# YifanXu74/MQ-Det

Measured on AMD Instinct MI355X. Metric: images/sec MQ-GLIP-T 800×1333 5-shot vision queries, 1/2/4/8 MI355X, higher is better.
Workload: dtype f16; 1 GPU; BASELINE.json configs[1]: MQ-GLIP-T (Swin-T + BERT-base + GCP + 6-layer VLDyHead), 5 vision queries x 40 classes, 141-token caption, LVIS-style post-processing; every step a full forward (feature / language caches OFF; only host-side tokenizer / query-selection results are memoised)); global_batch=8, batch_per_gpu=8, image=800x1333 -> 800x1344, parallelism=dp1, weights=seeded random init (no checkpoints offline), residual_streams=fp32

## Files before the change

### include/mqdet_hip.h

```cpp
#ifndef MQDET_HIP_H
#define MQDET_HIP_H
#ifdef __cplusplus
extern "C" {
#endif

int mq_abi_version(void);

long mq_attn_workspace_bytes(int B, int H, int Nq, int D, int nsplit);
int mq_attn_fwd(const void* q, const void* k, const void* vt, void* o, const float* key_bias, const int* kv_len,
                const unsigned char* qk_mask, long mask_bs, long mask_hs, long mask_rs, void* workspace,
                int B, int H, int Nq, int Nk, int D,
                long q_bs, long q_rs, long q_hs, long k_bs, long k_rs, long k_hs, long vt_bs, long vt_rs, long vt_hs,
                long o_bs, long o_rs, long bias_bs, long bias_hs, float scale, float clamp, int nsplit, void* stream);

int mq_attn_resident_fwd(const void* q, const void* k, const void* vt, void* o, const float* key_bias, const int* kv_len,
                         const unsigned char* qk_mask, long mask_bs, long mask_hs, long mask_rs, int B, int H, int Nq, int Nk, int D,
                         long q_bs, long q_rs, long q_hs, long k_bs, long k_rs, long k_hs, long vt_bs, long vt_rs, long vt_hs,
                         long o_bs, long o_rs, long bias_bs, long bias_hs, float scale, float clamp, void* stream);

int mq_attn_chunked_fwd(const void* q, const void* k, const void* vt, void* o, const float* key_bias, const int* kv_len,
                        void* workspace, int B, int H, int Nq, int Nk, int D,
                        long q_bs, long q_rs, long q_hs, long k_bs, long k_rs, long k_hs, long vt_bs, long vt_rs, long vt_hs,
                        long o_bs, long o_rs, long bias_bs, long bias_hs, float scale, float clamp, int nsplit, void* stream);

// ... 12 lines not shown
                      const void* out_bias, void* out, int B, int N, int T, int heads, int max_kv, float clamp, int variant,
                      void* stream);

long mq_vlfuse_t2i_workspace_bytes(int B, int T, int nsplit);
int mq_vlfuse_t2i_fwd(const void* kf, long kv_bs, long kv_hs, long kv_ts, const void* v_ln, const int* kv_len, const unsigned char* key_mask,
                      long key_mask_bs, void* workspace, void* out, int B, int N, int T, int heads, int nsplit, int max_kv, float clamp, int variant,
                      void* stream);

int mq_layernorm_fwd(const void* x, int x_f32, const void* res, int res_f32, const void* gamma, const void* beta, void* y,
                     float* y32, void* xsum, long rows, int C, float eps, void* stream);

int mq_layernorm2_fwd(const void* x, int x_f32, const void* res, int res_f32, const void* gamma, const void* beta, void* y,
                     float* y32, void* xsum, long rows, int C, float eps, void* stream);
int mq_layernorm_clamp_fwd(const void* x, int x_f32, const void* res, int res_f32, const void* gamma, const void* beta, void* y, float* y32,
                           void* xsum, long rows, int C, float eps, float clamp, void* stream);
int mq_clamp_gelu_clamp(const void* x, void* out, long n, float clamp, void* stream);

int mq_patch_merge_ln_fwd(const void* x, int x_f32, const void* gamma, const void* beta, void* y, int B, int H, int W, int C, float eps,
                          void* stream);

int mq_swin_mlp2_fwd(const float* x, const void* delta, const void* ln_g, const void* ln_b, float eps, const void* w1f,
                     const void* b1, const void* w2f, const void* b2, float* out, const void* next_g, const void* next_b,
                     float eps_next, void* y, long M, int C, int flags, void* stream);

int mq_conv3x3_fwd(const void* x, const void* w, const void* bias, void* out, int B, int H, int W, int C, long x_bs,
                   int N, int out_ld, int stride, void* stream);
int mq_conv3x3_nchw32_fwd(const void* x, const void* w, const void* bias, float* out, int B, int H, int W, int C, long x_bs,
                          int N, void* stream);

int mq_conv3x3_nchw32_v2_fwd(const void* x, const void* w, const void* bias, float* out, int B, int H, int W, int C, long x_bs,
                          int N, void* stream);
typedef struct mq_conv_level {
  const void* x; float* out; long x_bs; int H, W;
} mq_conv_level;
int mq_conv3x3_nchw32_group_fwd(const mq_conv_level* levels, int nl, const void* w, const void* bias, int B, int C, int N, void* stream);
int mq_pool2x2_tokens_fwd(const mq_conv_level* levels, int nl, void* out, int B, int C, void* stream);
int mq_dcnv2_stats_blocks(int H, int W, int stride);
typedef struct mq_dcn_branch {
  const void* x; const float* om; const void* w; const void* bias; void* out; float* stats; const float* wy; const float* wx;
  long x_bs;
  int B, H, W, C, oH, oW, N, out_ld, stride, flags;
} mq_dcn_branch;
int mq_dcnv2_group_fwd(const mq_dcn_branch* branches, int n, void* stream);
int mq_dcnv2_fwd(const void* x, const float* om, const void* w, const void* bias, void* out, float* stats, const float* wy,
                 const float* wx, int B, int H, int W, int C, long x_bs, int oH, int oW, int N, int out_ld, int stride,
                 int flags, void* stream);
// ... 102 lines not shown
#define MQ_BF16_TWIN(name) extern decltype(name) name##_bf16;
#else
#define MQ_BF16_TWIN(name) extern __typeof__(name) name##_bf16;
#endif
MQ_BF16_TWIN(mq_attn_fwd)
MQ_BF16_TWIN(mq_attn_resident_fwd)
MQ_BF16_TWIN(mq_attn_text_fwd)
MQ_BF16_TWIN(mq_bert_attn_qkv_fwd)
MQ_BF16_TWIN(mq_patch_embed_fwd)
MQ_BF16_TWIN(mq_attn_chunked_fwd)
MQ_BF16_TWIN(mq_window_attn_fwd)
MQ_BF16_TWIN(mq_window_attn_qkv_fwd)
MQ_BF16_TWIN(mq_gcp_sparse_attn_fwd)
MQ_BF16_TWIN(mq_gcp_gate_residual_fwd)
MQ_BF16_TWIN(mq_gcp_attn_fwd)
MQ_BF16_TWIN(mq_vlfuse_i2t_fwd)
MQ_BF16_TWIN(mq_vlfuse_t2i_fwd)
MQ_BF16_TWIN(mq_layernorm_fwd)
MQ_BF16_TWIN(mq_layernorm2_fwd)
MQ_BF16_TWIN(mq_layernorm_clamp_fwd)
MQ_BF16_TWIN(mq_clamp_gelu_clamp)
MQ_BF16_TWIN(mq_patch_merge_ln_fwd)
MQ_BF16_TWIN(mq_swin_mlp2_fwd)
MQ_BF16_TWIN(mq_conv3x3_fwd)
MQ_BF16_TWIN(mq_conv3x3_nchw32_fwd)
MQ_BF16_TWIN(mq_conv3x3_nchw32_v2_fwd)
MQ_BF16_TWIN(mq_conv3x3_nchw32_group_fwd)
MQ_BF16_TWIN(mq_dcnv2_fwd)
MQ_BF16_TWIN(mq_dcnv2_group_fwd)
MQ_BF16_TWIN(mq_dyconv_stats)
MQ_BF16_TWIN(mq_dyconv_coef)
MQ_BF16_TWIN(mq_dyconv_coef_group)
MQ_BF16_TWIN(mq_dyconv_fuse)
MQ_BF16_TWIN(mq_dyrelu_coef)
MQ_BF16_TWIN(mq_dyconv_epilogue_group)
MQ_BF16_TWIN(mq_dyrelu_apply)
MQ_BF16_TWIN(mq_add_upsample_nearest)
MQ_BF16_TWIN(mq_pool2x2_tokens_fwd)
MQ_BF16_TWIN(mq_dyrelu_ln_fwd)
MQ_BF16_TWIN(mq_align_scores_fwd)
MQ_BF16_TWIN(mq_align_fused_fwd)
MQ_BF16_TWIN(mq_box_decode)
MQ_BF16_TWIN(mq_roi_align_fwd)
MQ_BF16_TWIN(mq_msdeform_attn_fwd)
MQ_BF16_TWIN(mq_msdeform_attn_q_fwd)

// ... 51 lines not shown
```

### mq_det_amd/build.py

```python
import os
import subprocess
import sys

HERE = os.path.dirname(os.path.abspath(__file__))
CSRC = os.path.join(HERE, "csrc")
LIB_DIR = os.path.join(HERE, "lib")
LIB = os.path.join(LIB_DIR, "libmqdet_hip.so")
SOURCES = ["api.hip", "attn.hip", "attn_resident.hip", "attn_text.hip", "bert_attn.hip", "vlfuse_attn.hip", "window_attn.hip", "patch_embed.hip", "gcp.hip", "gcp_fused.hip", "conv_igemm.hip", "conv_small.hip", "conv_small2.hip", "conv_small3.hip", "dcn_fused.hip", "layernorm.hip", "layernorm2.hip", "dyconv.hip", "post.hip", "post2.hip", "align_fused.hip", "nms2.hip", "roi_align.hip", "swin_mlp2.hip", "msda.hip", "tta.hip", "lvis_eval.hip", "query_bank.hip"]
F32_SKIP = ("roi_align.hip", "nms2.hip", "post2.hip", "tta.hip", "lvis_eval.hip", "query_bank.hip")
FLAGS = ["--offload-arch=gfx950", "-O3", "-std=c++17", "-fPIC"]
EXTRA_FLAGS = {"dcn_fused.hip": ["-fno-slp-vectorize"],
               "swin_mlp2.hip": ["-fno-slp-vectorize"],
               "attn_resident.hip": ["-fno-slp-vectorize", "-mllvm", "-amdgpu-mfma-vgpr-form"],
               "attn_text.hip": ["-fno-slp-vectorize", "-mllvm", "-amdgpu-mfma-vgpr-form"],
               "bert_attn.hip": ["-fno-slp-vectorize", "-mllvm", "-amdgpu-mfma-vgpr-form"]}


STAMP = os.path.join(LIB_DIR, "libmqdet_hip.stamp")


def _digest():
    import hashlib
    h = hashlib.sha256()
    deps = sorted(os.path.join(CSRC, f) for f in os.listdir(CSRC)) + [os.path.join(HERE, "..", "include", "mqdet_hip.h"), os.path.abspath(__file__)]
    for d in deps:
        if os.path.isfile(d):
            with open(d, "rb") as f:
                h.update(os.path.basename(d).encode() + b"\0" + f.read())
    return h.hexdigest()


def _stale():
    if not os.path.exists(LIB) or not os.path.exists(STAMP):
        return True
    with open(STAMP) as f:
# ... 36 lines not shown
```

### mq_det_amd/modeling/pipeline.py

```python
import math
import os

import torch
import torch.nn.functional as F

from .. import ops

NEG = -1.0e30


def _pack_swin(P, sd, SW, p, device, dtype):
    def h(name):
        return sd[name].detach().to(device=device, dtype=dtype).contiguous()
    ws = SW.WINDOW_SIZE
    N = ws * ws
    for i, (depth, heads) in enumerate(zip(SW.DEPTHS, SW.NUM_HEADS)):
        for j in range(depth):
            b = f"{p}.layers.{i}.blocks.{j}.attn"
            idx = sd[b + ".relative_position_index"].to(device).reshape(-1)
            rel = sd[b + ".relative_position_bias_table"].detach().to(device=device, dtype=torch.float32)[idx]
            rel = rel.reshape(N, N, heads).permute(2, 0, 1)
            NP = ops.window_pad(ws)
            P[b + ".rel_bias"] = F.pad(rel, (0, NP - N, 0, NP - N)).contiguous()
    P["_swin_fused_mlp"] = bool(SW.get("FUSED_MLP", True)) and P["_r32"] and ops.KERNELS["SWIN_MLP_VARIANT"] == 2
    P["_swin_fused_widths"] = tuple(w for w in SW.get("FUSED_MLP_WIDTHS", ops.SWIN_MLP_WIDTHS) if w in ops.SWIN_MLP_WIDTHS)
    for i, depth in enumerate(SW.DEPTHS):
        Ci = SW.EMBED_DIM * 2 ** i
        if P["_swin_fused_mlp"] and Ci in P["_swin_fused_widths"]:
            for j in range(depth):
                b = f"{p}.layers.{i}.blocks.{j}.mlp"
                P[b + ".w1f"], P[b + ".w2f"] = ops.swin_mlp2_pack(h(b + ".fc1.weight"), h(b + ".fc2.weight"))
    w = sd[p + ".patch_embed.proj.weight"].detach().to(device=device, dtype=torch.float32)
    P[p + ".patch_embed.lin"] = w.permute(0, 2, 3, 1).reshape(w.shape[0], -1).to(dtype).contiguous()
    if w.shape[0] in (96, 192) and tuple(w.shape[1:]) == (3, 4, 4):
        P[p + ".patch_embed.wpk"] = ops.patch_embed_pack(w).to(dtype).contiguous()
        P[p + ".patch_embed.wpk_nchw"] = ops.patch_embed_pack(w, nchw=True).to(dtype).contiguous()
        P[p + ".patch_embed.f32"] = [sd[n].detach().to(device=device, dtype=torch.float32).contiguous() for n in
                                     (p + ".patch_embed.proj.bias", p + ".patch_embed.norm.weight", p + ".patch_embed.norm.bias",
                                      p + ".layers.0.blocks.0.norm1.weight", p + ".layers.0.blocks.0.norm1.bias")]


def _pack_language(P, sd, cfg, p, device, dtype):
    def h(name):
        return sd[name].detach().to(device=device, dtype=dtype).contiguous()

    def f32(name):
        return sd[name].detach().to(device=device, dtype=torch.float32).contiguous()
    LB = cfg.MODEL.LANGUAGE_BACKBONE
    nl = LB.get("NUM_HIDDEN_LAYERS", 12)
    for i in range(nl):
        _pack_bert_layer(P, sd, f"{p}.encoder.layer.{i}", device, dtype)
    if cfg.VISION_QUERY.ENABLED:
        qv0 = LB.get("QV_START", 6)
        for i in range(nl - qv0):
# ... 186 lines not shown
        x = _ln(P, p + ".patch_embed.norm", x, want_y=not r32, want_y32=r32)
    outs = []
    for i, (depth, heads) in enumerate(zip(M.DEPTHS, M.NUM_HEADS)):
        C = x.shape[-1]
        fused = P["_swin_fused_mlp"] and C in P["_swin_fused_widths"] and x.dtype == torch.float32
        pend = None
        h1 = None
        if i == 0 and h1_first is not None:
            h1 = h1_first
        for j in range(depth):
            b = f"{p}.layers.{i}.blocks.{j}"
            shift = 0 if j % 2 == 0 else ws // 2
            if h1 is None:
                if pend is None:
                    h1 = _ln(P, b + ".norm1", x)
                else:
                    h1, x = _add_ln(P, b + ".norm1", pend, x)
            if ops.window_qkv_fused(C, ws, h1.numel()):
                a = ops.window_attention_qkv(h1.reshape(B, H, W, C), P[b + ".attn.qkv.weight"], P[b + ".attn.qkv.bias"],
                                             P[b + ".attn.rel_bias"], heads, ws, shift)
            else:
                qkv = _lin(P, b + ".attn.qkv", h1).reshape(B, H, W, 3 * C)
                a = ops.window_attention(qkv, P[b + ".attn.qkv.bias"], P[b + ".attn.rel_bias"], heads, ws, shift)
            proj = _lin(P, b + ".attn.proj", a.reshape(B, H * W, C))
            if fused:
                nxt = f"{p}.layers.{i}.blocks.{j + 1}.norm1" if j + 1 < depth else (f"{p}.norm{i}" if i > 0 else None)
                nln = None if nxt is None else (P[nxt + ".weight"], P[nxt + ".bias"], 1e-5)
                r = ops.swin_mlp2(x.contiguous(), proj.contiguous(), P[b + ".norm2.weight"], P[b + ".norm2.bias"], 1e-5,
                                  P[b + ".mlp.w1f"], P[b + ".mlp.fc1.bias"], P[b + ".mlp.w2f"], P[b + ".mlp.fc2.bias"], next_ln=nln)
                x, h1 = r if nxt is not None else (r, None)
                pend = None
            else:
                h2, x = _add_ln(P, b + ".norm2", proj, x)
                pend = _lin(P, b + ".mlp.fc2", F.gelu(_lin(P, b + ".mlp.fc1", h2)))
                h1 = None
        if fused:
            if i > 0:
                outs.append(h1.reshape(B, H, W, C))
        elif i > 0:
            o, x = _add_ln(P, f"{p}.norm{i}", pend, x)
            outs.append(o.reshape(B, H, W, C))
        else:
            x = x + pend
        if i < len(M.DEPTHS) - 1:
            d = f"{p}.layers.{i}.downsample"
            if ops.KERNELS["PATCH_MERGE_FUSED"] == 1:
                yn = ops.patch_merge_ln(x.reshape(B, H, W, C).contiguous(), P[d + ".norm.weight"], P[d + ".norm.bias"], 1e-5)
                H, W = (H + 1) // 2, (W + 1) // 2
            else:
                y = x.reshape(B, H, W, C)
                if H % 2 or W % 2:
                    y = F.pad(y, (0, 0, 0, W % 2, 0, H % 2))
# ... 647 lines not shown
```

### mq_det_amd/ops.py

```python
import ctypes
import math
import os

import torch

_LIB = None
_LIB_PATH = os.path.join(os.path.dirname(os.path.abspath(__file__)), "lib", "libmqdet_hip.so")

_vp, _i, _l, _f = ctypes.c_void_p, ctypes.c_int, ctypes.c_long, ctypes.c_float
EXPECTED_ABI = 31
_SIGNATURES = {
    "mq_abi_version": (_i, []),
    "mq_attn_workspace_bytes": (_l, [_i, _i, _i, _i, _i]),
    "mq_attn_fwd": (_i, [_vp, _vp, _vp, _vp, _vp, _vp, _vp, _l, _l, _l, _vp, _i, _i, _i, _i, _i] + [_l] * 13 + [_f, _f, _i, _vp]),
    "mq_attn_resident_fwd": (_i, [_vp, _vp, _vp, _vp, _vp, _vp, _vp, _l, _l, _l, _i, _i, _i, _i, _i] + [_l] * 13 + [_f, _f, _vp]),
    "mq_patch_embed_fwd": (_i, [_vp, _i, _vp, _vp, _vp, _vp, _vp, _vp, _vp, _vp, _i, _i, _i, _i, _f, _vp]),
    "mq_attn_text_fwd": (_i, [_vp, _vp, _vp, _vp, _vp, _vp, _i, _i, _i, _i, _i] + [_l] * 13 + [_f, _f, _i, _vp]),
    "mq_bert_attn_qkv_fwd": (_i, [_vp, _vp, _vp, _vp, _vp, _vp, _i, _i, _i, _i, _l, _l, _l, _l, _l, _f, _f, _vp]),
    "mq_attn_chunked_fwd": (_i, [_vp, _vp, _vp, _vp, _vp, _vp, _vp, _i, _i, _i, _i, _i] + [_l] * 13 + [_f, _f, _i, _vp]),
    "mq_window_attn_fwd": (_i, [_vp, _vp, _vp, _vp, _i, _i, _i, _i, _i, _i, _i, _vp]),
    "mq_window_attn_qkv_fwd": (_i, [_vp, _vp, _vp, _vp, _vp, _i, _i, _i, _i, _i, _i, _i, _vp]),
    "mq_gcp_sparse_attn_fwd": (_i, [_vp, _vp, _vp, _vp, _i, _i, _i, _i, _i, _i, _vp]),
    "mq_gcp_gate_residual_fwd": (_i, [_vp, _vp, _vp, _vp, _i, _vp, _vp, _l, _i, _i, _vp]),
    "mq_gcp_attn_fwd": (_i, [_vp] * 16 + [_l, _i, _i, _i, _i, _i, _i, _i, _f, _i, _vp]),
    "mq_vlfuse_i2t_fwd": (_i, [_vp, _vp, _vp, _l, _l, _l, _vp, _vp, _vp, _vp, _i, _i, _i, _i, _i, _f, _i, _vp]),
    "mq_vlfuse_t2i_workspace_bytes": (_l, [_i, _i, _i]),
    "mq_vlfuse_t2i_fwd": (_i, [_vp, _l, _l, _l, _vp, _vp, _vp, _l, _vp, _vp, _i, _i, _i, _i, _i, _i, _f, _i, _vp]),
    "mq_layernorm_fwd": (_i, [_vp, _i, _vp, _i, _vp, _vp, _vp, _vp, _vp, _l, _i, _f, _vp]),
    "mq_layernorm2_fwd": (_i, [_vp, _i, _vp, _i, _vp, _vp, _vp, _vp, _vp, _l, _i, _f, _vp]),
    "mq_layernorm_clamp_fwd": (_i, [_vp, _i, _vp, _i, _vp, _vp, _vp, _vp, _vp, _l, _i, _f, _f, _vp]),
    "mq_clamp_gelu_clamp": (_i, [_vp, _vp, _l, _f, _vp]),
    "mq_patch_merge_ln_fwd": (_i, [_vp, _i, _vp, _vp, _vp, _i, _i, _i, _i, _f, _vp]),
    "mq_swin_mlp2_fwd": (_i, [_vp, _vp, _vp, _vp, _f, _vp, _vp, _vp, _vp, _vp, _vp, _vp, _f, _vp, _l, _i, _i, _vp]),
    "mq_conv3x3_fwd": (_i, [_vp, _vp, _vp, _vp, _i, _i, _i, _i, _l, _i, _i, _i, _vp]),
    "mq_conv3x3_nchw32_fwd": (_i, [_vp, _vp, _vp, _vp, _i, _i, _i, _i, _l, _i, _vp]),
    "mq_conv3x3_nchw32_v2_fwd": (_i, [_vp, _vp, _vp, _vp, _i, _i, _i, _i, _l, _i, _vp]),
    "mq_conv3x3_nchw32_group_fwd": (_i, [_vp, _i, _vp, _vp, _i, _i, _i, _vp]),
    "mq_dcnv2_stats_blocks": (_i, [_i, _i, _i]),
    "mq_dcnv2_fwd": (_i, [_vp, _vp, _vp, _vp, _vp, _vp, _vp, _vp, _i, _i, _i, _i, _l, _i, _i, _i, _i, _i, _i, _vp]),
    "mq_dcnv2_group_fwd": (_i, [_vp, _i, _vp]),
    "mq_dyconv_stats": (_i, [_vp, _vp, _vp, _vp, _i, _i, _i, _i, _vp]),
    "mq_dyconv_coef": (_i, [_vp, _vp, _vp, _vp, _vp, _vp, _i, _i, _i, _i, _i, _f, _i, _vp]),
    "mq_dyconv_coef_group": (_i, [_vp, _i, _vp, _vp, _i, _i, _i, _f, _vp]),
    "mq_dyconv_fuse": (_i, [_vp, _vp, _i, _i, _vp, _vp, _i, _i, _vp, _vp, _i, _i, _i, _vp, _l, _vp, _i, _i, _i, _i, _vp]),
    "mq_dyrelu_coef": (_i, [_vp, _vp, _vp, _vp, _vp, _vp, _i, _i, _i, _vp]),
    "mq_dyconv_epilogue_group": (_i, [_vp, _i, _vp, _vp, _vp, _vp, _i, _i, _vp]),
    "mq_add_upsample_nearest": (_i, [_vp, _vp, _i, _i, _i, _i, _i, _i, _vp]),
    "mq_pool2x2_tokens_fwd": (_i, [_vp, _i, _vp, _i, _i, _vp]),
    "mq_dyrelu_ln_fwd": (_i, [_vp, _l, _vp, _vp, _i, _vp, _vp, _f, _vp, _i, _i, _i, _vp]),
    "mq_dyrelu_apply": (_i, [_vp, _vp, _i, _i, _i, _l, _vp]),
    "mq_align_scores_fwd": (_i, [_vp, _i, _vp, _vp, _l, _vp, _vp, _vp, _i, _i, _i, _i, _i, _f, _l, _i, _vp]),
    "mq_align_fused_fwd": (_i, [_vp, _vp, _vp, _vp, _vp, _vp, _vp, _l, _vp, _vp, _vp, _vp, _vp, _vp, _i, _i, _i, _i, _i, _i, _i, _f, _i, _vp]),
    "mq_box_decode": (_i, [_vp, _vp, _vp, _i, _vp, _vp, _l, _vp, _vp, _vp, _vp, _i, _i, _i, _i, _l, _l, _vp]),
    "mq_roi_align_fwd": (_i, [_vp, _i, _vp, _vp, _i, _i, _i, _i, _l, _l, _l, _l, _i, _i, _f, _i, _i, _i, _vp]),
    "mq_msdeform_attn_fwd": (_i, [_vp, _i, _vp, _vp, _vp, _vp, _vp, _i, _i, _i, _i, _i, _i, _i, _i, _vp]),
    "mq_msdeform_attn_q_fwd": (_i, [_vp, _i, _l, _l, _vp, _vp, _vp, _vp, _i, _vp, _vp, _i, _i, _i, _i, _i, _i, _i, _i, _vp]),
    "mq_post_select_workspace_bytes": (_l, [_vp, _vp, _i, _i, _i]),
    "mq_post_select_fwd": (_i, [_vp, _vp, _vp, _vp, _vp, _i, _i, _i, _vp, _l, _vp, _vp, _vp, _vp, _vp, _vp, _vp]),
    "mq_post_sort_fwd": (_i, [_vp, _vp, _vp, _vp, _i, _vp, _vp, _vp, _vp, _i, _i, _vp]),
    "mq_post_finalize_fwd": (_i, [_vp, _vp, _vp, _vp, _vp, _vp, _i, _i, _i, _i, _vp]),
    "mq_ml_nms_workspace_bytes": (_l, [_i, _i]),
    "mq_ml_nms_topk": (_i, [_vp, _vp, _vp, _vp, _vp, _i, _i, _f, _i, _vp]),
    "mq_ml_nms": (_i, [_vp, _vp, _vp, _vp, _vp, _i, _i, _f, _vp]),
    "mq_tta_ingest_fwd": (_i, [_vp] * 8 + [_i] * 5 + [_vp, _vp, _i, _i, _vp]),
    "mq_tta_merge_prep": (_i, [_vp] * 5 + [_i] + [_vp] * 10 + [_i, _i, _i, _vp]),
    "mq_tta_merge_finalize": (_i, [_vp] * 12 + [_i, _i, _i, _vp]),
    "mq_lvis_match": (_i, [_vp] * 13 + [_i, _l, _vp]),
    "mq_lvis_accumulate": (_i, [_vp] * 7 + [_i, _vp]),
    "mq_bank_admit": (_i, [_vp] * 8 + [_i] * 8 + [_f, _vp]),
}
BF16_TWINS = ("mq_attn_fwd", "mq_attn_resident_fwd", "mq_attn_text_fwd", "mq_bert_attn_qkv_fwd", "mq_patch_embed_fwd", "mq_attn_chunked_fwd", "mq_window_attn_fwd", "mq_window_attn_qkv_fwd", "mq_gcp_sparse_attn_fwd", "mq_gcp_gate_residual_fwd", "mq_gcp_attn_fwd", "mq_vlfuse_i2t_fwd", "mq_vlfuse_t2i_fwd",
              "mq_layernorm_fwd", "mq_layernorm2_fwd", "mq_layernorm_clamp_fwd", "mq_clamp_gelu_clamp", "mq_patch_merge_ln_fwd", "mq_swin_mlp2_fwd", "mq_conv3x3_fwd", "mq_conv3x3_nchw32_fwd", "mq_conv3x3_nchw32_v2_fwd", "mq_conv3x3_nchw32_group_fwd", "mq_dcnv2_fwd", "mq_dcnv2_group_fwd",
              "mq_dyconv_stats", "mq_dyconv_coef", "mq_dyconv_coef_group", "mq_dyconv_fuse", "mq_dyrelu_coef", "mq_dyconv_epilogue_group", "mq_dyrelu_apply", "mq_dyrelu_ln_fwd", "mq_add_upsample_nearest", "mq_pool2x2_tokens_fwd",
              "mq_align_scores_fwd", "mq_align_fused_fwd", "mq_box_decode", "mq_roi_align_fwd", "mq_msdeform_attn_fwd", "mq_msdeform_attn_q_fwd")
F32_TWINS = tuple(n for n in BF16_TWINS if n not in ("mq_roi_align_fwd",))
for _n in BF16_TWINS:
    _SIGNATURES[_n + "_bf16"] = _SIGNATURES[_n]
for _n in F32_TWINS:
    _SIGNATURES[_n + "_f32"] = _SIGNATURES[_n]
EXPORTS = tuple(_SIGNATURES)


from .selection import KERNEL_DEFAULTS, KERNELS, _ThreadLocalTable, configure, activate


def lib_path():
    return _LIB_PATH


def load_library():
    global _LIB
    if _LIB is None:
        if not os.path.exists(_LIB_PATH):
            raise RuntimeError(f"{_LIB_PATH} not found: the MI355X HIP library is required (python -m mq_det_amd.build); "
                               "there is no CPU / eager fallback for the MQ-Det hot path")
        lib = ctypes.CDLL(_LIB_PATH)
        for name, (res, args) in _SIGNATURES.items():
            fn = getattr(lib, name)
# ... 582 lines not shown
    if auto:
        flags = 3 if C < 384 else 2
    if f32_operands():
        flags = 0 if auto else flags & ~2
    fn = _fn(lib, "mq_swin_mlp2_fwd", w1f)

    def call(fl):
        _chk(fn(_ptr(x), _ptr(delta), _ptr(ln_g), _ptr(ln_b), float(eps), _ptr(w1f), _ptr(b1), _ptr(w2f), _ptr(b2),
                _ptr(out), _ptr(ng), _ptr(nb), float(ne), _ptr(y), M, C, fl, _stream()), "mq_swin_mlp2_fwd")
    side = _tail_stream(x.device) if (KERNELS["SWIN_MLP_TAIL_STREAM"] == 1 and x.is_cuda and not (flags & 29) and _TIMING is None) else None
    with _timed(f"swin_mlp_c{C}", M * C * (4 + 4 + (2 if delta is not None else 0) + (2 if y is not None else 0))):
        if side is None:
            call(flags)
        else:
            main = torch.cuda.current_stream()
            side.wait_stream(main)
            with torch.cuda.stream(side):
                call(flags | 16)
            call(flags | 8)
            main.wait_stream(side)
    return (out, y) if y is not None else out


_TAIL_STREAMS = {}


def _tail_stream(device):
    s = _TAIL_STREAMS.get(device.index)
    if s is None:
        s = _TAIL_STREAMS[device.index] = torch.cuda.Stream(device=device)
    return s


def conv3x3(x_nhwc, w_packed, bias, n_out, stride=1):
    lib = load_library()
    _need_gpu(x_nhwc, w_packed, bias)
    B, H, W, C = x_nhwc.shape
    assert x_nhwc.dtype in _H16 and x_nhwc.stride(3) == 1 and x_nhwc.stride(2) == C and x_nhwc.stride(1) == W * C
    assert w_packed.is_contiguous() and w_packed.shape == (32 if n_out <= 32 else 256, 9 * C) and w_packed.dtype == x_nhwc.dtype
    Ho, Wo = (H + 2 - 3) // stride + 1, (W + 2 - 3) // stride + 1
    ld = n_out if n_out % 8 == 0 else (n_out + 7) // 8 * 8
    out = torch.empty(B, Ho, Wo, ld, dtype=x_nhwc.dtype, device=x_nhwc.device)
    with _timed("conv3x3"):
        _chk(_fn(lib, "mq_conv3x3_fwd", x_nhwc)(_ptr(x_nhwc), _ptr(w_packed), _ptr(bias), _ptr(out), B, H, W, C, x_nhwc.stride(0), n_out, ld,
                                stride, _stream()), "mq_conv3x3_fwd")
    return out if ld == n_out else out[..., :n_out]
# ... 684 lines not shown
```

### mq_det_amd/selection.py

```python
import os

KERNEL_DEFAULTS = {
    "LN_VARIANT": 2,
    "OFFSET_CONV_VARIANT": 3,
    "PATCH_MERGE_FUSED": 1,
    "FPN_VIA_DCN": 1,
    "NMS_EARLY_STOP": 1,
    "ATTN_RESIDENT": 1,
    "SWIN_MLP_VARIANT": 2,
    "SWIN_MLP2_FLAGS": -1,
    "SWIN_QKV_FUSED": 2,
    "FPN_TOPDOWN_FUSED": 1,
    "DYRELU_IN_LN": 1,
    "VLFUSE_I2T_VARIANT": 0,
    "SWIN_MLP_TAIL_STREAM": 0,
    "DYCONV_EPILOGUE_GROUPED": 1,
    "BERT_CLAMP_FUSED": 1,
    "PATCH_EMBED_FUSED": 1,
    "BERT_QKV_FUSED": 1,
    "FRONT_SIDE_STREAM": 1,
    "LANG_SIDE_STREAMS": 0,
    "GCP_ATTN_FUSED": 1,
    "BERT_ATTN_QKV_FUSED": 1,
    "POST_FUSED": 1,
    "F32_OPERANDS": 0,
    "DCN_BDMA": 1,
    "POOLED_TOKENS_FUSED": 1,
    "ALIGN_FUSED": 1,
}
class _ThreadLocalTable(dict):

    def __init__(self, init):
        super().__init__()
# ... 66 lines not shown
```

Measured before the change: 493.9 images/sec.

## Fuse Swin attention output projection into the fused MLP kernel

Adds a swin_mlp2p kernel that computes the attention output projection (with bias and residual add) inside the fused LN+MLP kernel for C=96/192 stages, so the projection result no longer round-trips through global memory as a separate GEMM. The projection weights are staged through LDS before the MLP pipeline, and fc1 columns are permuted at pack time to match. Rows left over by the wave-quantization split go to the existing tail kernel after a host-side linear. It is enabled by default and adds extra LDS staging and register pressure to the main kernel.

New measurement: 499.8 images/sec, median of 6. Within noise of the previous version (+1.2%).

```diff
diff --git a/include/mqdet_hip.h b/include/mqdet_hip.h
--- a/include/mqdet_hip.h
+++ b/include/mqdet_hip.h
@@ -58,6 +58,11 @@
 int mq_swin_mlp2_fwd(const float* x, const void* delta, const void* ln_g, const void* ln_b, float eps, const void* w1f,
                      const void* b1, const void* w2f, const void* b2, float* out, const void* next_g, const void* next_b,
                      float eps_next, void* y, long M, int C, int flags, void* stream);
+
+long mq_swin_mlp2p_main_rows(long M, int C, int flags);
+int mq_swin_mlp2p_fwd(const float* x, const void* a, const void* wpf, const void* bp, const void* ln_g, const void* ln_b, float eps,
+                      const void* w1fp, const void* b1, const void* w2f, const void* b2, float* out, const void* next_g, const void* next_b,
+                      float eps_next, void* y, const void* w1f, const void* delta_tail, long M, int C, int flags, void* stream);
 
 int mq_conv3x3_fwd(const void* x, const void* w, const void* bias, void* out, int B, int H, int W, int C, long x_bs,
                    int N, int out_ld, int stride, void* stream);
@@ -206,6 +211,7 @@
 MQ_BF16_TWIN(mq_clamp_gelu_clamp)
 MQ_BF16_TWIN(mq_patch_merge_ln_fwd)
 MQ_BF16_TWIN(mq_swin_mlp2_fwd)
+MQ_BF16_TWIN(mq_swin_mlp2p_fwd)
 MQ_BF16_TWIN(mq_conv3x3_fwd)
 MQ_BF16_TWIN(mq_conv3x3_nchw32_fwd)
 MQ_BF16_TWIN(mq_conv3x3_nchw32_v2_fwd)
diff --git a/mq_det_amd/build.py b/mq_det_amd/build.py
--- a/mq_det_amd/build.py
+++ b/mq_det_amd/build.py
@@ -6,11 +6,12 @@
 CSRC = os.path.join(HERE, "csrc")
 LIB_DIR = os.path.join(HERE, "lib")
 LIB = os.path.join(LIB_DIR, "libmqdet_hip.so")
-SOURCES = ["api.hip", "attn.hip", "attn_resident.hip", "attn_text.hip", "bert_attn.hip", "vlfuse_attn.hip", "window_attn.hip", "patch_embed.hip", "gcp.hip", "gcp_fused.hip", "conv_igemm.hip", "conv_small.hip", "conv_small2.hip", "conv_small3.hip", "dcn_fused.hip", "layernorm.hip", "layernorm2.hip", "dyconv.hip", "post.hip", "post2.hip", "align_fused.hip", "nms2.hip", "roi_align.hip", "swin_mlp2.hip", "msda.hip", "tta.hip", "lvis_eval.hip", "query_bank.hip"]
-F32_SKIP = ("roi_align.hip", "nms2.hip", "post2.hip", "tta.hip", "lvis_eval.hip", "query_bank.hip")
+SOURCES = ["api.hip", "attn.hip", "attn_resident.hip", "attn_text.hip", "bert_attn.hip", "vlfuse_attn.hip", "window_attn.hip", "patch_embed.hip", "gcp.hip", "gcp_fused.hip", "conv_igemm.hip", "conv_small.hip", "conv_small2.hip", "conv_small3.hip", "dcn_fused.hip", "layernorm.hip", "layernorm2.hip", "dyconv.hip", "post.hip", "post2.hip", "align_fused.hip", "nms2.hip", "roi_align.hip", "swin_mlp2.hip", "swin_mlp2p.hip", "msda.hip", "tta.hip", "lvis_eval.hip", "query_bank.hip"]
+F32_SKIP = ("roi_align.hip", "nms2.hip", "post2.hip", "tta.hip", "lvis_eval.hip", "query_bank.hip", "swin_mlp2p.hip")
 FLAGS = ["--offload-arch=gfx950", "-O3", "-std=c++17", "-fPIC"]
 EXTRA_FLAGS = {"dcn_fused.hip": ["-fno-slp-vectorize"],
                "swin_mlp2.hip": ["-fno-slp-vectorize"],
+               "swin_mlp2p.hip": ["-fno-slp-vectorize"],
                "attn_resident.hip": ["-fno-slp-vectorize", "-mllvm", "-amdgpu-mfma-vgpr-form"],
                "attn_text.hip": ["-fno-slp-vectorize", "-mllvm", "-amdgpu-mfma-vgpr-form"],
                "bert_attn.hip": ["-fno-slp-vectorize", "-mllvm", "-amdgpu-mfma-vgpr-form"]}
diff --git a/mq_det_amd/csrc/swin_mlp2p.hip b/mq_det_amd/csrc/swin_mlp2p.hip
--- /dev/null
+++ b/mq_det_amd/csrc/swin_mlp2p.hip
@@ -0,0 +1,382 @@
+#include "common.h"
+#include <type_traits>
+
+#if !defined(MQ_F32)
+
+MQ_NAMESPACE_BEGIN
+
+extern "C" int MQ_SYM(mq_swin_mlp2_fwd)(const float* x, const void* delta, const void* ln_g, const void* ln_b, float eps, const void* w1f,
+                                        const void* b1, const void* w2f, const void* b2, float* out, const void* next_g, const void* next_b,
+                                        float eps_next, void* y, long M, int C, int flags, void* stream);
+
+struct SwinMlp2pParams {
+  const float* x; const half_t* a;
+  const half_t* wpf; const half_t* bp;
+  const half_t* g2; const half_t* be2;
+  const half_t* w1fp; const half_t* b1; const half_t* w2f; const half_t* b2;
+  float* out;
+  const half_t* gn; const half_t* bn; half_t* y;
+  long M; float eps, eps_n;
+};
+
+__device__ __forceinline__ float erf_abs_scaled_p(float v) {
+  const float t = __builtin_amdgcn_rcpf(fmaf(0.3275911f * 0.70710678118654752f, fabsf(v), 1.f));
+  const float poly = t * (0.254829592f + t * (-0.284496736f + t * (1.421413741f + t * (-1.453152027f + t * 1.061405429f))));
+  const float ex = __builtin_amdgcn_exp2f((-0.5f * 1.4426950408889634f) * v * v);
+  return fmaf(-poly, ex, 1.f);
+}
+template <int I, int N, class F>
+__device__ __forceinline__ void static_for_p_impl(F& f) {
+  if constexpr (I < N) {
+    f(std::integral_constant<int, I>{});
+    static_for_p_impl<I + 1, N>(f);
+  }
+}
+template <int N, class F>
+__device__ __forceinline__ void static_for_p(F f) { static_for_p_impl<0, N>(f); }
+constexpr int gelu_piece_of_p(int q, int GS, bool want_k) {
+  int c = 0;
+  for (int d = 0; d < 8 + GS - 1; ++d)
+    for (int st = 0; st < GS; ++st) {
+      const int k = d - st;
+      if (k < 0 || k >= 8) continue;
+      if (c == q) return want_k ? k : st;
+      ++c;
+    }
+  return -1;
+}
+#define MQ_GELU_TAB_N 768
+
+template <int C, int NW, bool TABLE>
+__global__ __launch_bounds__(64 * NW, C <= 96 ? 4 : 3) void swin_mlp2p_kernel(SwinMlp2pParams p) {
+  constexpr int NT = 64 * NW, BM = 16 * NW, HID = 4 * C, KS = C / 32, CT = C / 16, NCHUNK = HID / 32;
+  constexpr int FR = 512;
+  constexpr int W1_FR = 2 * KS, W2_FR = CT, IT_FR = W1_FR + W2_FR;
+  constexpr int FPW = IT_FR / NW;
+  constexpr int D = 1, NS = D + 1, U = 2;
+  constexpr int PT = NS * IT_FR / KS, NR = (CT + PT - 1) / PT;
+  static_assert(C % 32 == 0 && C <= 192 && IT_FR % NW == 0 && NCHUNK % U == 0, "tile shapes");
+  extern __shared__ __attribute__((aligned(16))) char smem[];
+  half_t* w1s = (half_t*)smem;
+  half_t* w2s = w1s + NS * W1_FR * FR;
+  half_t* b1s = w2s + NS * W2_FR * FR;
+  float* tab = (float*)(b1s + HID);
+
+  const int tid = threadIdx.x, lane = tid & 63, l15 = lane & 15, g = lane >> 4;
+  const int wave = __builtin_amdgcn_readfirstlane(tid >> 6);
+  const long row0 = (long)blockIdx.x * BM + wave * 16;
+
+  const mq_rsrc rs_w1 = mq_raw_buffer(p.w1fp), rs_w2 = mq_raw_buffer(p.w2f), rs_wp = mq_raw_buffer(p.wpf);
+  auto stage_issue = [&](int c1, int s1, int c2, int s2) __attribute__((always_inline)) {
+#pragma unroll
+    for (int i = 0; i < FPW; ++i) {
+      const int f = wave + i * NW;
+      const mq_rsrc rs = f < W1_FR ? rs_w1 : rs_w2;
+      const int eoff = f < W1_FR ? (c1 * W1_FR + f) * FR : (c2 * W2_FR + (f - W1_FR)) * FR;
+      half_t* dst = f < W1_FR ? w1s + (s1 * W1_FR + f) * FR : w2s + (s2 * W2_FR + (f - W1_FR)) * FR;
+      lds_stage_frag8_buf(rs, nullptr, eoff, lane * 8, dst, lane);
+    }
+  };
+
+  const long row = min(row0 + l15, p.M - 1);
+  half8 af[KS];
+#pragma unroll
+  for (int ks = 0; ks < KS; ++ks) af[ks] = *(const half8*)(p.a + row * C + ks * 32 + g * 8);
+  float4_ xr[CT];
+#pragma unroll
+  for (int ct = 0; ct < CT; ++ct) xr[ct] = *(const float4_*)(p.x + row * C + ct * 16 + 4 * g);
+
+  float4_ acc2[CT];
+#pragma unroll
+  for (int ct = 0; ct < CT; ++ct) acc2[ct] = (float4_){0.f, 0.f, 0.f, 0.f};
+
+  static_for_p<NR>([&](auto rc) __attribute__((always_inline)) {
+    constexpr int rd = decltype(rc)::value, T0 = rd * PT, NTL = (CT - T0) < PT ? (CT - T0) : PT, NB = NTL * KS;
+    if constexpr (rd > 0) __syncthreads();
+#pragma unroll
+    for (int i = 0; i < (NB + NW - 1) / NW; ++i) {
+      const int f = wave + i * NW;
+      if (f < NB) lds_stage_frag8_buf(rs_wp, nullptr, (T0 * KS + f) * FR, lane * 8, w1s + f * FR, lane);
+    }
+    if constexpr (rd == 0) {
+      for (int i = tid; i < HID / 8; i += NT) *(half8*)(b1s + i * 8) = *(const half8*)(p.b1 + i * 8);
+      if constexpr (TABLE) {
+        for (int i = tid; i < MQ_GELU_TAB_N; i += NT) {
+          const float x0 = -6.f + (float)i * (1.f / 64.f), x1 = x0 + (1.f / 64.f);
+          const float p0 = fmaf(0.5f, __builtin_copysignf(erf_abs_scaled_p(x0), x0), 0.5f);
+          const float p1 = fmaf(0.5f, __builtin_copysignf(erf_abs_scaled_p(x1), x1), 0.5f);
+          tab[2 * i] = p0;
+          tab[2 * i + 1] = p1 - p0;
+        }
+      }
+    }
+    asm volatile("s_waitcnt vmcnt(0)" ::: "memory");
+    __syncthreads();
+#pragma unroll
+    for (int t = 0; t < NTL; ++t)
+#pragma unroll
+      for (int ks = 0; ks < KS; ++ks) acc2[T0 + t] = mfma16(*(const half8*)(w1s + (t * KS + ks) * FR + lane * 8), af[ks], acc2[T0 + t]);
+  });
+  __syncthreads();
+#pragma unroll
+  for (int c = 0; c <= D; ++c) stage_issue(c, c % NS, 0, c == 0 ? 0 : NS - 1);
+
+  half8 xf[KS];
+  {
+    float s = 0.f;
+#pragma unroll
+    for (int ct = 0; ct < CT; ++ct) {
+      const half4 bpv = *(const half4*)(p.bp + ct * 16 + 4 * g);
+#pragma unroll
+      for (int r = 0; r < 4; ++r) {
+        const half_t d = (half_t)(acc2[ct][r] + (float)bpv[r]);
+        acc2[ct][r] = xr[ct][r] + (float)d;
+        s += acc2[ct][r];
+      }
+    }
+    s += __shfl_xor(s, 16);
+    s += __shfl_xor(s, 32);
+    const float mean = s * (1.f / (float)C);
+    float q = 0.f;
+#pragma unroll
+    for (int ct = 0; ct < CT; ++ct)
+#pragma unroll
+      for (int r = 0; r < 4; ++r) { const float d = acc2[ct][r] - mean; q += d * d; }
+    q += __shfl_xor(q, 16);
+    q += __shfl_xor(q, 32);
+    const float rstd = rsqrtf(q * (1.f / (float)C) + p.eps);
+#pragma unroll
+    for (int ct = 0; ct < CT; ++ct) {
+      const int c = ct * 16 + 4 * g;
+      const half4 gm = *(const half4*)(p.g2 + c), bt = *(const half4*)(p.be2 + c), b2 = *(const half4*)(p.b2 + c);
+#pragma unroll
+      for (int r = 0; r < 4; ++r) {
+        xf[ct >> 1][4 * (ct & 1) + r] = (half_t)((acc2[ct][r] - mean) * rstd * (float)gm[r] + (float)bt[r]);
+        acc2[ct][r] += (float)b2[r];
+      }
+    }
+  }
+
+  asm volatile("s_waitcnt vmcnt(0)" ::: "memory");
+  __syncthreads();
+
+  auto h_init = [&](int c, float4_ (&h)[2]) __attribute__((always_inline)) {
+    const int hb = min(c, NCHUNK - 1) * 32 + 4 * g;
+    const half4 b0 = *(const half4*)(b1s + hb), b1 = *(const half4*)(b1s + hb + 16);
+#pragma unroll
+    for (int r = 0; r < 4; ++r) { h[0][r] = (float)b0[r]; h[1][r] = (float)b1[r]; }
+  };
+  auto gemm1 = [&](int st, float4_ (&h)[2]) {
+    const half_t* a = w1s + st * W1_FR * FR + lane * 8;
+#pragma unroll
+    for (int ks = 0; ks < KS; ++ks) {
+      h[0] = mfma16(*(const half8*)(a + ks * FR), xf[ks], h[0]);
+      h[1] = mfma16(*(const half8*)(a + (KS + ks) * FR), xf[ks], h[1]);
+    }
+  };
+  auto gemm2 = [&](int st, const half8& hf) {
+    const half_t* a = w2s + st * W2_FR * FR + lane * 8;
+#pragma unroll
+    for (int ct = 0; ct < CT; ++ct) acc2[ct] = mfma16(*(const half8*)(a + ct * FR), hf, acc2[ct]);
+  };
+
+  constexpr int RD = 6, GS = TABLE ? 2 : 3, NPIECE = 8 * GS;
+#define MQ_PIN(x) asm volatile("" : "+v"(x))
+  auto gelu_piece = [&](auto kc, auto stc, const float4_ (&hin)[2], half8& hf, float (&gts)[8], float (&ges)[8], float (&gds)[8]) __attribute__((always_inline)) {
+    constexpr int k = decltype(kc)::value, stage = decltype(stc)::value;
+    float& gt = gts[k];
+    float& ge = ges[k];
+    float v = hin[k >> 2][k & 3];
+    MQ_PIN(v);
+    if constexpr (TABLE) {
+      if constexpr (stage == 0) {
+        const float pos = fmaf(__builtin_amdgcn_fmed3f(v, -6.f, 5.9921875f), 64.f, 384.f);
+        const int idx = (int)pos;
+        gt = pos - (float)idx;
+        MQ_PIN(gt);
+        const float2_ e = *(const float2_*)(tab + 2 * idx);
+        ge = e[0];
+        gds[k] = e[1];
+      } else {
+        float t = gt * gds[k];
+        MQ_PIN(t);
+        float o = v * (t + ge);
+        MQ_PIN(o);
+        hf[k] = (half_t)o;
+      }
+    } else {
+      (void)gds;
+      if constexpr (stage == 0) {
+        gt = __builtin_amdgcn_rcpf(fmaf(0.3275911f * 0.70710678118654752f, fabsf(v), 1.f));
+        ge = __builtin_amdgcn_exp2f((-0.5f * 1.4426950408889634f) * v * v);
+        MQ_PIN(gt);
+        MQ_PIN(ge);
+      } else if constexpr (stage == 1) {
+        const float t = gt;
+        gt = t * (0.254829592f + t * (-0.284496736f + t * (1.421413741f + t * (-1.453152027f + t * 1.061405429f))));
+        MQ_PIN(gt);
+      } else {
+        const float hv = 0.5f * v;
+        float o = fmaf(hv, __builtin_copysignf(fmaf(-gt, ge, 1.f), v), hv);
+        MQ_PIN(o);
+        hf[k] = (half_t)o;
+      }
+    }
+  };
+  auto step = [&](int j, auto PHc, float4_ (&hin)[2], float4_ (&hout)[2], half8& hf_old, half8& hf_new) __attribute__((always_inline)) {
+    constexpr int PH = decltype(PHc)::value;
+    constexpr int N = 2 * KS + CT;
+    constexpr int S1 = (PH + 1) % NS, S2 = (PH + NS - 1) % NS;
+    stage_issue(min(j + 1 + D, NCHUNK + 1), PH, min(j - 1 + D, NCHUNK - 1), (PH + NS - 2) % NS);
+    h_init(j + 1, hout);
+    const half_t* a1 = w1s + S1 * W1_FR * FR + lane * 8;
+    const half_t* a2 = w2s + S2 * W2_FR * FR + lane * 8;
+    auto frag = [&](int i) __attribute__((always_inline)) -> half8 {
+      const int m = i >> 1;
+      return (i & 1) ? *(const half8*)(a2 + m * FR) : *(const half8*)(a1 + ((m & 1) * KS + (m >> 1)) * FR);
+    };
+    half8 ring[RD];
+    float gts[8], ges[8], gds[8];
+#pragma unroll
+    for (int i = 0; i < RD && i < N; ++i) ring[i] = frag(i);
+    static_for_p<N>([&](auto ic) __attribute__((always_inline)) {
+      constexpr int i = decltype(ic)::value;
+      static_for_p<NPIECE>([&](auto qc) __attribute__((always_inline)) {
+        constexpr int q = decltype(qc)::value;
+        if constexpr (q * N / NPIECE == i)
+          gelu_piece(std::integral_constant<int, gelu_piece_of_p(q, GS, true)>{}, std::integral_constant<int, gelu_piece_of_p(q, GS, false)>{},
+                     hin, hf_new, gts, ges, gds);
+      });
+      const half8 a = ring[i % RD];
+      if constexpr (!(i & 1)) {
+        constexpr int m = i >> 1;
+        hout[m & 1] = mfma16(a, xf[m >> 1], hout[m & 1]);
+      } else {
+        acc2[i >> 1] = mfma16(a, hf_old, acc2[i >> 1]);
+      }
+      if constexpr (i + RD < N) ring[i % RD] = frag(i + RD);
+      __builtin_amdgcn_sched_barrier(0);
+    });
+    asm volatile("s_waitcnt vmcnt(%0)" ::"n"((D - 1) * FPW) : "memory");
+    __builtin_amdgcn_s_barrier();
+  };
+  float4_ hA[2], hB[2];
+  half8 hfA, hfB = zero8();
+  h_init(0, hA);
+  gemm1(0, hA);
+  __syncthreads();
+  for (int jb = 0; jb < NCHUNK; jb += U)
+    static_for_p<U>([&](auto uc) __attribute__((always_inline)) {
+      constexpr int u = decltype(uc)::value;
+      if constexpr (u % 2 == 0)
+        step(jb + u, std::integral_constant<int, u % NS>{}, hA, hB, hfB, hfA);
+      else
+        step(jb + u, std::integral_constant<int, u % NS>{}, hB, hA, hfA, hfB);
+    });
+  gemm2((NCHUNK - 1) % NS, hfB);
+  asm volatile("s_waitcnt vmcnt(0)" ::: "memory");
+#undef MQ_PIN
+
+  {
+    const long orow = row0 + l15;
+    const bool live = orow < p.M;
+    float s = 0.f;
+#pragma unroll
+    for (int ct = 0; ct < CT; ++ct) {
+#pragma unroll
+      for (int r = 0; r < 4; ++r) s += acc2[ct][r];
+      if (live) *(float4_*)(p.out + orow * C + ct * 16 + 4 * g) = acc2[ct];
+    }
+    if (p.y) {
+      s += __shfl_xor(s, 16);
+      s += __shfl_xor(s, 32);
+      const float mean = s * (1.f / (float)C);
+      float q = 0.f;
+#pragma unroll
+      for (int ct = 0; ct < CT; ++ct)
+#pragma unroll
+        for (int r = 0; r < 4; ++r) { const float d = acc2[ct][r] - mean; q += d * d; }
+      q += __shfl_xor(q, 16);
+      q += __shfl_xor(q, 32);
+      const float rstd = rsqrtf(q * (1.f / (float)C) + p.eps_n);
+      if (live) {
+#pragma unroll
+        for (int ct = 0; ct < CT; ++ct) {
+          const int c = ct * 16 + 4 * g;
+          const half4 gm = *(const half4*)(p.gn + c), bt = *(const half4*)(p.bn + c);
+          half4 o;
+#pragma unroll
+          for (int r = 0; r < 4; ++r) o[r] = (half_t)((acc2[ct][r] - mean) * rstd * (float)gm[r] + (float)bt[r]);
+          *(half4*)(p.y + orow * C + c) = o;
+        }
+      }
+    }
+  }
+}
+
+template <int C, int NW, bool TABLE>
+static int launch_swin_mlp2p_main(const SwinMlp2pParams& p, hipStream_t s) {
+  constexpr size_t smem = (size_t)(2 * 2 * (C / 32) + 2 * (C / 16)) * 512 * sizeof(half_t) + (size_t)4 * C * sizeof(half_t) +
+                          (TABLE ? MQ_GELU_TAB_N * 2 * sizeof(float) : 0);
+  static MqOncePerDevice attr;
+  if (attr.first()) {
+    hipError_t e = hipFuncSetAttribute((const void*)swin_mlp2p_kernel<C, NW, TABLE>, hipFuncAttributeMaxDynamicSharedMemorySize, (int)smem);
+    if (e != hipSuccess) return (int)e;
+    attr.done();
+  }
+  constexpr int BM = 16 * NW;
+  hipLaunchKernelGGL((swin_mlp2p_kernel<C, NW, TABLE>), dim3((unsigned)((p.M + BM - 1) / BM)), dim3(64 * NW), smem, s, p);
+  MQ_CHECK_LAUNCH();
+  return 0;
+}
+
+template <int NW, int WPC>
+static long swin_mlp2p_main_rows(long M, int flags) {
+  constexpr int BM = 16 * NW;
+  if (flags & 1) return M;
+  const long cus = mq_device_cus(), wgs = (M + BM - 1) / BM, slots = cus * WPC, rem = wgs % slots;
+  return (wgs > slots && rem > 0 && rem * NW <= 2L * cus) ? (wgs - rem) * BM : M;
+}
+static long swin_mlp2p_main_rows_c(long M, int C, int flags) {
+  switch (C) {
+    case 96: return swin_mlp2p_main_rows<4, 4>(M, flags);
+    case 192: return swin_mlp2p_main_rows<4, 3>(M, flags);
+    default: return -1;
+  }
+}
+
+#if defined(MQ_PRIMARY_UNIT)
+extern "C" long mq_swin_mlp2p_main_rows(long M, int C, int flags) { return M <= 0 ? 0 : swin_mlp2p_main_rows_c(M, C, flags); }
+#endif
+
+extern "C" int MQ_SYM(mq_swin_mlp2p_fwd)(const float* x, const void* a, const void* wpf, const void* bp, const void* ln_g, const void* ln_b,
+                                         float eps, const void* w1fp, const void* b1, const void* w2f, const void* b2, float* out,
+                                         const void* next_g, const void* next_b, float eps_next, void* y, const void* w1f,
+                                         const void* delta_tail, long M, int C, int flags, void* stream) {
+  if (M <= 0) return 0;
+  if (y && (!next_g || !next_b)) return -2;
+  const long m_main = swin_mlp2p_main_rows_c(M, C, flags);
+  if (m_main < 0) return -1;
+  if (m_main < M) {
+    if (!w1f || !delta_tail) return -3;
+    const int e = MQ_SYM(mq_swin_mlp2_fwd)(x + m_main * C, delta_tail, ln_g, ln_b, eps, w1f, b1, w2f, b2, out + m_main * C, next_g, next_b,
+                                           eps_next, y ? (void*)((half_t*)y + m_main * C) : nullptr, M - m_main, C, 4, stream);
+    if (e) return e;
+  }
+  if (m_main == 0) return 0;
+  SwinMlp2pParams p;
+  p.x = x; p.a = (const half_t*)a; p.wpf = (const half_t*)wpf; p.bp = (const half_t*)bp; p.g2 = (const half_t*)ln_g; p.be2 = (const half_t*)ln_b;
+  p.eps = eps; p.w1fp = (const half_t*)w1fp; p.b1 = (const half_t*)b1; p.w2f = (const half_t*)w2f; p.b2 = (const half_t*)b2; p.out = out;
+  p.gn = (const half_t*)next_g; p.bn = (const half_t*)next_b; p.eps_n = eps_next; p.y = (half_t*)y; p.M = m_main;
+  hipStream_t s = (hipStream_t)stream;
+  const bool table = flags & 2;
+  switch (C) {
+    case 96: return table ? launch_swin_mlp2p_main<96, 4, true>(p, s) : launch_swin_mlp2p_main<96, 4, false>(p, s);
+    case 192: return table ? launch_swin_mlp2p_main<192, 4, true>(p, s) : launch_swin_mlp2p_main<192, 4, false>(p, s);
+    default: return -1;
+  }
+}
+
+MQ_NAMESPACE_END
+
+#endif
diff --git a/mq_det_amd/modeling/pipeline.py b/mq_det_amd/modeling/pipeline.py
--- a/mq_det_amd/modeling/pipeline.py
+++ b/mq_det_amd/modeling/pipeline.py
@@ -30,6 +30,16 @@
             for j in range(depth):
                 b = f"{p}.layers.{i}.blocks.{j}.mlp"
                 P[b + ".w1f"], P[b + ".w2f"] = ops.swin_mlp2_pack(h(b + ".fc1.weight"), h(b + ".fc2.weight"))
+    P["_swin_proj_fused_widths"] = ()
+    if P["_swin_fused_mlp"] and ops.KERNELS.get("SWIN_PROJ_FUSED", 0) == 1 and torch.device(device).type == "cuda" \
+            and dtype in (torch.float16, torch.bfloat16) and not ops.f32_operands():
+        P["_swin_proj_fused_widths"] = tuple(w for w in P["_swin_fused_widths"] if w in ops.SWIN_PROJ_FUSED_WIDTHS)
+        for i, depth in enumerate(SW.DEPTHS):
+            if SW.EMBED_DIM * 2 ** i in P["_swin_proj_fused_widths"]:
+                for j in range(depth):
+                    b = f"{p}.layers.{i}.blocks.{j}"
+                    P[b + ".attn.proj.wpf"], P[b + ".mlp.w1fp"], _ = ops.swin_mlp2p_pack(h(b + ".attn.proj.weight"), h(b + ".mlp.fc1.weight"),
+                                                                                      h(b + ".mlp.fc2.weight"))
     w = sd[p + ".patch_embed.proj.weight"].detach().to(device=device, dtype=torch.float32)
     P[p + ".patch_embed.lin"] = w.permute(0, 2, 3, 1).reshape(w.shape[0], -1).to(dtype).contiguous()
     if w.shape[0] in (96, 192) and tuple(w.shape[1:]) == (3, 4, 4):
@@ -262,12 +272,20 @@
             else:
                 qkv = _lin(P, b + ".attn.qkv", h1).reshape(B, H, W, 3 * C)
                 a = ops.window_attention(qkv, P[b + ".attn.qkv.bias"], P[b + ".attn.rel_bias"], heads, ws, shift)
-            proj = _lin(P, b + ".attn.proj", a.reshape(B, H * W, C))
+            pfused = fused and x.is_cuda and C in P.get("_swin_proj_fused_widths", ()) and a.dtype == P[b + ".mlp.w2f"].dtype
+            if not pfused:
+                proj = _lin(P, b + ".attn.proj", a.reshape(B, H * W, C))
             if fused:
                 nxt = f"{p}.layers.{i}.blocks.{j + 1}.norm1" if j + 1 < depth else (f"{p}.norm{i}" if i > 0 else None)
                 nln = None if nxt is None else (P[nxt + ".weight"], P[nxt + ".bias"], 1e-5)
-                r = ops.swin_mlp2(x.contiguous(), proj.contiguous(), P[b + ".norm2.weight"], P[b + ".norm2.bias"], 1e-5,
-                                  P[b + ".mlp.w1f"], P[b + ".mlp.fc1.bias"], P[b + ".mlp.w2f"], P[b + ".mlp.fc2.bias"], next_ln=nln)
+                if pfused:
+                    r = ops.swin_mlp2p(x.contiguous(), a.reshape(B, H * W, C).contiguous(), P[b + ".attn.proj.wpf"], P[b + ".attn.proj.bias"],
+                                       P[b + ".norm2.weight"], P[b + ".norm2.bias"], 1e-5, P[b + ".mlp.w1fp"], P[b + ".mlp.fc1.bias"],
+                                       P[b + ".mlp.w2f"], P[b + ".mlp.fc2.bias"], next_ln=nln,
+                                       tail=(P[b + ".attn.proj.weight"], P[b + ".mlp.w1f"]))
+                else:
+                    r = ops.swin_mlp2(x.contiguous(), proj.contiguous(), P[b + ".norm2.weight"], P[b + ".norm2.bias"], 1e-5,
+                                      P[b + ".mlp.w1f"], P[b + ".mlp.fc1.bias"], P[b + ".mlp.w2f"], P[b + ".mlp.fc2.bias"], next_ln=nln)
                 x, h1 = r if nxt is not None else (r, None)
                 pend = None
             else:
diff --git a/mq_det_amd/ops.py b/mq_det_amd/ops.py
--- a/mq_det_amd/ops.py
+++ b/mq_det_amd/ops.py
@@ -32,6 +32,8 @@
     "mq_clamp_gelu_clamp": (_i, [_vp, _vp, _l, _f, _vp]),
     "mq_patch_merge_ln_fwd": (_i, [_vp, _i, _vp, _vp, _vp, _i, _i, _i, _i, _f, _vp]),
     "mq_swin_mlp2_fwd": (_i, [_vp, _vp, _vp, _vp, _f, _vp, _vp, _vp, _vp, _vp, _vp, _vp, _f, _vp, _l, _i, _i, _vp]),
+    "mq_swin_mlp2p_main_rows": (_l, [_l, _i, _i]),
+    "mq_swin_mlp2p_fwd": (_i, [_vp] * 6 + [_f] + [_vp] * 7 + [_f, _vp, _vp, _vp, _l, _i, _i, _vp]),
     "mq_conv3x3_fwd": (_i, [_vp, _vp, _vp, _vp, _i, _i, _i, _i, _l, _i, _i, _i, _vp]),
     "mq_conv3x3_nchw32_fwd": (_i, [_vp, _vp, _vp, _vp, _i, _i, _i, _i, _l, _i, _vp]),
     "mq_conv3x3_nchw32_v2_fwd": (_i, [_vp, _vp, _vp, _vp, _i, _i, _i, _i, _l, _i, _vp]),
@@ -70,10 +72,10 @@
     "mq_bank_admit": (_i, [_vp] * 8 + [_i] * 8 + [_f, _vp]),
 }
 BF16_TWINS = ("mq_attn_fwd", "mq_attn_resident_fwd", "mq_attn_text_fwd", "mq_bert_attn_qkv_fwd", "mq_patch_embed_fwd", "mq_attn_chunked_fwd", "mq_window_attn_fwd", "mq_window_attn_qkv_fwd", "mq_gcp_sparse_attn_fwd", "mq_gcp_gate_residual_fwd", "mq_gcp_attn_fwd", "mq_vlfuse_i2t_fwd", "mq_vlfuse_t2i_fwd",
-              "mq_layernorm_fwd", "mq_layernorm2_fwd", "mq_layernorm_clamp_fwd", "mq_clamp_gelu_clamp", "mq_patch_merge_ln_fwd", "mq_swin_mlp2_fwd", "mq_conv3x3_fwd", "mq_conv3x3_nchw32_fwd", "mq_conv3x3_nchw32_v2_fwd", "mq_conv3x3_nchw32_group_fwd", "mq_dcnv2_fwd", "mq_dcnv2_group_fwd",
+              "mq_layernorm_fwd", "mq_layernorm2_fwd", "mq_layernorm_clamp_fwd", "mq_clamp_gelu_clamp", "mq_patch_merge_ln_fwd", "mq_swin_mlp2_fwd", "mq_swin_mlp2p_fwd", "mq_conv3x3_fwd", "mq_conv3x3_nchw32_fwd", "mq_conv3x3_nchw32_v2_fwd", "mq_conv3x3_nchw32_group_fwd", "mq_dcnv2_fwd", "mq_dcnv2_group_fwd",
               "mq_dyconv_stats", "mq_dyconv_coef", "mq_dyconv_coef_group", "mq_dyconv_fuse", "mq_dyrelu_coef", "mq_dyconv_epilogue_group", "mq_dyrelu_apply", "mq_dyrelu_ln_fwd", "mq_add_upsample_nearest", "mq_pool2x2_tokens_fwd",
               "mq_align_scores_fwd", "mq_align_fused_fwd", "mq_box_decode", "mq_roi_align_fwd", "mq_msdeform_attn_fwd", "mq_msdeform_attn_q_fwd")
-F32_TWINS = tuple(n for n in BF16_TWINS if n not in ("mq_roi_align_fwd",))
+F32_TWINS = tuple(n for n in BF16_TWINS if n not in ("mq_roi_align_fwd", "mq_swin_mlp2p_fwd"))
 for _n in BF16_TWINS:
     _SIGNATURES[_n + "_bf16"] = _SIGNATURES[_n]
 for _n in F32_TWINS:
@@ -702,6 +704,49 @@
     return (out, y) if y is not None else out
 
 
+SWIN_PROJ_FUSED_WIDTHS = (96, 192)
+
+
+def swin_mlp2p_pack(wp, w1, w2):
+    C = wp.shape[0]
+    assert wp.shape == (C, C) and w1.shape == (4 * C, C) and C in SWIN_PROJ_FUSED_WIDTHS and not f32_operands()
+    wpf = wp.reshape(C // 16, 16, C // 32, 4, 8).permute(0, 2, 3, 1, 4).reshape(-1).contiguous()
+    w1fp, w2f = swin_mlp2_pack(w1[:, swin_mlp_w2_perm(C, w1.device)], w2)
+    return wpf, w1fp, w2f
+
+
+def swin_mlp2p(x, a, wpf, bp, ln_g, ln_b, eps, w1fp, b1, w2f, b2, next_ln=None, flags=None, tail=None):
+    lib = load_library()
+    _need_gpu(x, a, wpf, bp, ln_g, ln_b, w1fp, b1, w2f, b2)
+    C = x.shape[-1]
+    M = x.numel() // C
+    h16 = wpf.dtype
+    assert C in SWIN_PROJ_FUSED_WIDTHS and not f32_operands() and x.dtype == torch.float32 and x.is_contiguous()
+    assert a.dtype == h16 and a.is_contiguous() and a.numel() == x.numel() and h16 in (torch.float16, torch.bfloat16)
+    assert wpf.numel() == C * C and w1fp.numel() == (4 * C // 32 + 2) * (C // 16) * 512 and w2f.numel() == (4 * C // 32) * (C // 16) * 512
+    assert all(t.is_contiguous() and t.dtype == h16 for t in (wpf, bp, ln_g, ln_b, w1fp, b1, w2f, b2))
+    out = torch.empty_like(x)
+    y, ng, nb, ne = None, None, None, 0.0
+    if next_ln is not None:
+        ng, nb, ne = next_ln
+        y = torch.empty(x.shape, dtype=h16, device=x.device)
+    flags = KERNELS["SWIN_MLP2_FLAGS"] if flags is None else int(flags)
+    flags = 3 if flags < 0 else flags & 3
+    m_main = int(lib.mq_swin_mlp2p_main_rows(M, C, flags))
+    w1f = dtail = None
+    if m_main < M:
+        if tail is None:
+            raise ValueError("swin_mlp2p: the pass / tail split leaves rows for the tail kernel: pass tail=(attn.proj.weight, w1f)")
+        wp, w1f = tail
+        assert wp.dtype == w1f.dtype == h16 and w1f.is_contiguous() and w1f.numel() == w1fp.numel()
+        dtail = torch.nn.functional.linear(a.reshape(M, C)[m_main:], wp, bp).contiguous()
+    with _timed(f"swin_mlp2p_c{C}", M * C * (4 + 4 + 2 + (2 if y is not None else 0))):
+        _chk(_fn(lib, "mq_swin_mlp2p_fwd", wpf)(_ptr(x), _ptr(a), _ptr(wpf), _ptr(bp), _ptr(ln_g), _ptr(ln_b), float(eps), _ptr(w1fp), _ptr(b1),
+                                                _ptr(w2f), _ptr(b2), _ptr(out), _ptr(ng), _ptr(nb), float(ne), _ptr(y), _ptr(w1f), _ptr(dtail),
+                                                M, C, flags, _stream()), "mq_swin_mlp2p_fwd")
+    return (out, y) if y is not None else out
+
+
 _TAIL_STREAMS = {}
 
 
diff --git a/mq_det_amd/selection.py b/mq_det_amd/selection.py
--- a/mq_det_amd/selection.py
+++ b/mq_det_amd/selection.py
@@ -9,6 +9,7 @@
     "ATTN_RESIDENT": 1,
     "SWIN_MLP_VARIANT": 2,
     "SWIN_MLP2_FLAGS": -1,
+    "SWIN_PROJ_FUSED": 1,
     "SWIN_QKV_FUSED": 2,
     "FPN_TOPDOWN_FUSED": 1,
     "DYRELU_IN_LN": 1,
```
